# Daniel-Lin-S/decode_tonal_langauge

Hardware: AMD Instinct MI355X
Metric: mel-frames/sec (train step) SynthesisModelCNN, 128ch x 400t batch256 (higher is better)
Workload: dtype f32; 1 GPU; SynthesisModelCNN 128ch x 400t -> 80 mel, 4 tones x 2 syllables, L=5, global batch 256 (strong scaling: 256 windows on rank 0), dropout 0.5, NAdam, 1,376,768,720 params; per_gpu_batch=256, global_batch=256, parallelism=dp1, init=drawn on every rank

## Files before the change

decode_tonal_langauge_amd/_cnnrnn_classifier_train_engine.py:

```python
from __future__ import annotations

from typing import Optional

import torch
import torch.nn as nn

from . import _kernels
from ._classifier_engine import C_A, C_B, C_FIRST, K7, Conv7Trunk, geometry, lstm_pack, lstm_pack_buffers
from ._classifier_train_engine import SUPPORTED, ClassifierTrainEngine, check_common, refuse
from ._conv_stack import ConvStack
from ._launch import r4
from ._lib import EPI_MASK, EPI_STORE, LOAD_DIRECT, LOAD_V, LOAD_Y, check, ptr

def lstm2_input_index(b: int, ch: int, s: int, w: int, B: int, tq: int, W: int, channels: int = C_B):
    f = (ch * tq + s) * W + w
    return (f // (channels * W)) * B + b, f % (channels * W)


def check_supported(model) -> None:
    from .models.deep_classifiers import CNNRNNClassifier
    if not isinstance(model, CNNRNNClassifier):
        refuse(f"model {type(model).__name__}")
    tq = geometry(model.input_channels, model.input_length, model.lstm1.hidden_size)["tq"]
    check_common(model, [m.negative_slope for m in model.modules() if isinstance(m, nn.LeakyReLU)], float(model.conv_block3[5].p),
# ... 162 lines not shown
        rows, nhex, cin, cout = S * Tp, S * Tp // 6, st.cin, st.cout
        f32 = dict(dtype=torch.float32, device=self._dev)
        src, Gs = self.P[st.idx - 1], self.G[st.idx]
        tag = f"conv{st.idx}_wgrad"
        fwd_tag = "conv3a_fwd" if st.idx == 2 else "conv3b_fwd"
        kept = self._v7_of == (self.generation, fwd_tag)
        V0, V1 = (self._hex_view(v, cin, nhex) for v in self.V7)
        ev = self._tick(tag + "_xform")
        if not kept:
            check(self.lib.tl_wino63_xform2(ptr(src), ptr(V0), ptr(V1), rows, Tp, st.tin, cin, src.shape[1], cin, self._stream()),
                  "tl_wino63_xform2")
            self._v7_of = (self.generation, fwd_tag)
        Y = self._hex_view(self.Y7, cout, nhex)
        check(self.lib.tl_wino63_ydz(ptr(Gs), ptr(Y), rows, Tp, st.tout, cout, Gs.shape[1], cout, self._stream()), "tl_wino63_ydz")
        if ev:
            ev[1].record()
        sk = self._splitk((cin // 64) * (cout // 64), (rows + 35) // 36, 4096)
        slab = torch.empty(3, sk, 8 * cin, cout, **f32)
        bias_part = torch.empty(sk, cout, **f32)
        ev = self._tick(tag)
        for s, (V, a_hex) in enumerate(((V0, 0), (V1, 0), (V0, 1))):
            self._tn(fn="tl_conv3_wino63v_tn", A=ptr(V), B=ptr(Y), slab=ptr(slab[s]), Krows=rows, A_rows=V.shape[0],
                     B_rows=Y.shape[0], Mdim=cin, Ndim=cout, lda=cin, ldb=cout, ldc=cout, J=3, Tp=Tp, splitk=sk,
                     slab_stride=8 * cin * cout, loader=LOAD_Y, Tvalid=st.tout, a_hex=a_hex,
                     colsum=ptr(bias_part) if s == 0 else None)
        if ev:
            ev[1].record()
        n = 8 * cin * cout
        ev = self._tick(tag + "_reduce")
        red = torch.empty(8 * cin, cout, **f32) if sk > 1 else None
        g3 = torch.empty(cout, cin, 3, **f32)
        gw7 = gw.view(cout, cin, K7)
        for s in range(3):
            if sk > 1:
                self._permute(slab[s], red, (1, 1, 1, n), (0, 0, 0, 1), nz=sk, zs=n)
            check(self.lib.tl_wino63_wgrad_finalize(ptr(red if sk > 1 else slab[s]), ptr(g3), cout, cin, cout, self._stream()),
                  "tl_wino63_wgrad_finalize")
            nt = min(3, K7 - 3 * s)
            gw7[:, :, 3 * s:3 * s + nt].copy_(g3[:, :, :nt])
        self._permute(bias_part, gb, (1, 1, 1, cout), (0, 0, 0, 1), nz=sk, zs=cout)
        if ev:
            ev[1].record()

    def _dgrad7(self, st, w: torch.Tensor) -> None:
        S, Tp = self.S, self.Tp
        rows, nhex, cin, cout = S * Tp, S * Tp // 6, st.cin, st.cout
        Gs, out = self.G[st.idx], self.G[st.idx - 1]
# ... 95 lines not shown
```

decode_tonal_langauge_amd/_conv_stack.py:

```python
from __future__ import annotations

from typing import List

import torch

from . import _kernels, _lib
from ._launch import LaunchTimers, launch_nt, launch_tn, permute_reduce, r4
from ._lib import (EPI_C1WGRAD, EPI_GY, EPI_LRELU, EPI_MASK, EPI_MASKY, EPI_POOL, EPI_POOLV, LOAD_DIRECT, LOAD_UNPOOL, LOAD_V,
                   LOAD_Y, check, ptr)


class _Stage:

    def __init__(self, idx, cin, cout, k, pool, tin, tp_in):
        self.idx, self.cin, self.cout, self.k, self.pool = idx, cin, cout, k, pool
        self.tin, self.tp_in = tin, tp_in
        self.tc = tin - k + 1
        self.tout = self.tc // 2 if pool else self.tc
        self.tp_out = tp_in // 2 if pool else tp_in


class ConvStack(LaunchTimers):
    F63_CAPABLE = True

# ... 16 lines not shown
        self.tp1 = max(align, (self.tout1 + align - 1) // align * align)
        _kernels.validate()
        self.wino63 = (self.F63_CAPABLE and _kernels.get("wino") == "6"
                       and self._f63_covers(stage_defs, n_timepoints))
        tp1_default = self.tp1
        if self.wino63:
            self.tp1 = (self.tout1 + 11) // 12 * 12
        self.f63_yprod = (self.wino63 and _kernels.get("f63_yprod") != "0" and stage_defs[0][0] % 256 == 0
                          and self.tp1 >= 12)
        self.f63_yprod3 = (self.wino63 and _kernels.get("f63_yprod") != "0" and stage_defs[1][0] % 256 == 0)
        self.stages: List[_Stage] = []
        cin, tin, tp = self.c1, self.tout1, self.tp1
        for i, (cout, k, pool) in enumerate(stage_defs[1:], start=2):
            st = _Stage(i, cin, cout, k, pool, tin, tp)
            if st.tout < 1:
                raise ValueError("n_timepoints too small for the conv stack")
            if self.wino63 and i == 3:
                st.tp_out = tp1_default // 4
            self.stages.append(st)
            cin, tin, tp = cout, st.tout, st.tp_out
        self.gy4 = self._gy_applies()
        st3 = self.stages[1] if len(self.stages) >= 2 else None
        self.f63_seq16 = bool(self.wino63 and self.f63_yprod and self.f63_yprod3 and self.gy4
                              and _kernels.get("f63_yprod") == "1" and -(-st3.tc // 6) <= 16 < st3.tp_in // 6)
        self.lat = tin
        self.tp5 = tp
        self.ld5 = r4(conv_channels)
        mode = _kernels.get("wino")
        self.wino43 = mode != "0"
        self.store_p1 = _kernels.get("store_p1") == "1"
        self.fuse_c1 = True
        self.wino_vout = True
        self.tn_bm = 0
        self._gy_A = None
        self._vhalo = {}
        self._B = None
        self.generation = 0

    def _alloc(self, B: int, dev) -> bool:
        if self._B == B and self._dev == dev:
            return False
        self._B, self._dev = B, dev
        self.S = B * self.C
        self._v_ready = {}
        self._gy_A = None
        self._vhalo = {}
        self._alloc_rows()
# ... 142 lines not shown
        Pout = self.P.get(st.idx) if (st.idx != 2 or self.store_p1) else None
        kw = dict(A=ptr(V), A_rows=V.shape[0], lda=V.shape[2], loader=LOAD_V, Bw=ptr(wp), bias=ptr(bia), out=ptr(Pout),
                  M=S * st.tp_in, N=st.cout, K=st.cin, ldb=st.cin, ldo=Pout.shape[1] if Pout is not None else st.cout, J=3,
                  row_shift=0, Tp=st.tp_in, slope=self.slope, obits=ptr(self.bits[st.idx]), osign=ptr(self.sbits[st.idx]),
                  ld_obits=st.cout // 32, Tvalid=2 * st.tout)
        if st.idx == 2:
            rows_out = S * st.tp_out
            Vn = self._v_hex_buffer(self.V, 2, rows_out, st.cout)
            ntm = -(-(S * st.tp_in) // self._nt63_rows())
            halo = self._halo_buffer(2, ntm, st.cout)
            kw.update(epilogue=EPI_POOLV, vout=ptr(Vn), vhalo=ptr(halo), vout_quads=Vn.shape[0], ld_vout=Vn.shape[2])
            self._nt(tag="conv2_fwd", fn="tl_conv3_wino63v_nt", **kw)
            check(self.lib.tl_wino63_v_fixup(ptr(Vn), ptr(halo), rows_out // 6, ntm, st.tp_out, st.cout, Vn.shape[2],
                                             self._stream()), "tl_wino63_v_fixup")
            self._v_ready[2] = Vn
        else:
            if Pout is None:
                raise RuntimeError("F(6,3) stage 3 writes pooled rows: its output buffer was not allocated")
            kw.update(epilogue=EPI_POOL, out_tp=st.tp_out)
            if self._seq16(st):
                kw.update(M=S * 96, Tp=96, a_hps_extra=st.tp_in // 6 - 16)
            self._nt(tag="conv3_fwd", fn="tl_conv3_wino63v_nt", **kw)

    def _stage_wgrad63(self, st, gw, gb) -> None:
        S = self.S
        f32 = dict(dtype=torch.float32, device=self._dev)
        rows_in = S * st.tp_in
        nd = st.cout
        ldg = nd
        V = self._v_ready[st.idx - 1]
        tiles = (st.cin // 64) * (nd // 64)
        sk = self._splitk(tiles, (rows_in + 35) // 36, 4096)
        slab = torch.empty(sk, 8 * st.cin, ldg, **f32)
        bias_part = torch.empty(sk, nd, **f32)
        if (st.idx == 3 and self.f63_yprod3 and self._y_ready.get(3) != self.generation):
            Gs = self.G[3]
            Y3 = self._v_hex_buffer(self.Yt, 3, rows_in, nd)
            Vd3 = self._vd3_buffer(rows_in, nd)
            ev = self._tick("conv3_yvd")
            check(self.lib.tl_wino63_unpool_yvd(ptr(Gs), ptr(self.bits[3]), ptr(Y3), ptr(Vd3), rows_in, Gs.shape[0], st.tp_in,
                                                st.tp_out, 2 * st.tout, nd, Gs.shape[1], st.cout // 32, nd, self._stream()),
                  "tl_wino63_unpool_yvd")
            if ev:
                ev[1].record()
            self._y_ready[3] = self.generation
            self._vd_ready[3] = self.generation
        if self._y_ready.get(st.idx) == self.generation:
            Y = self.Yt[st.idx]
            self._y_ready[st.idx] = -1
            self._tn(tag=f"conv{st.idx}_wgrad", fn="tl_conv3_wino63v_tn", A=ptr(V), B=ptr(Y), slab=ptr(slab), Krows=rows_in,
                     A_rows=V.shape[0], B_rows=Y.shape[0], Mdim=st.cin, Ndim=nd, lda=V.shape[2], ldb=Y.shape[2], ldc=ldg, J=3,
                     Tp=st.tp_in, splitk=sk, slab_stride=8 * st.cin * ldg, loader=LOAD_Y, Tvalid=2 * st.tout,
                     colsum=ptr(bias_part))
        else:
            Gs = self.G[st.idx]
            Vd = self._v_hex_buffer(self.Vd, st.idx, rows_in, nd)
            self._tn(tag=f"conv{st.idx}_wgrad", fn="tl_conv3_wino63v_tn", A=ptr(V), B=ptr(Gs), slab=ptr(slab), Krows=rows_in,
                     A_rows=V.shape[0], B_rows=Gs.shape[0], Mdim=st.cin, Ndim=nd, lda=V.shape[2], ldb=Gs.shape[1], ldc=ldg, J=3,
                     Tp=st.tp_in, splitk=sk, slab_stride=8 * st.cin * ldg, loader=LOAD_UNPOOL, bbits=ptr(self.bits[st.idx]),
                     ld_bbits=st.cout // 32, Tvalid=2 * st.tout, colsum=ptr(bias_part), vd=ptr(Vd), ld_vd=nd, g_tp=st.tp_out)
            self._vd_ready[st.idx] = self.generation
        self._wino_wgrad_tail(st, slab, bias_part, 8, "tl_wino63_wgrad_finalize", gw, gb)

    def _wino_wgrad_tail(self, st, slab, bias_part, taps, finalize, gw, gb) -> None:
        sk, rows, ldg = slab.shape
        if sk > 1:
            red = torch.empty(rows, ldg, dtype=torch.float32, device=self._dev)
            n = taps * st.cin * ldg
            self._permute(slab, red, (1, 1, 1, n), (0, 0, 0, 1), nz=sk, zs=n)
        else:
            red = slab
        check(getattr(self.lib, finalize)(ptr(red), ptr(gw), st.cout, st.cin, ldg, self._stream()), finalize)
        self._permute(bias_part, gb, (1, 1, 1, st.cout), (0, 0, 0, 1), nz=sk, zs=bias_part.shape[1])

    def _gy_stage(self, st) -> bool:
# ... 435 lines not shown
```

decode_tonal_langauge_amd/_kernels.py:

```python
from __future__ import annotations

import os
from typing import Callable, Dict, Tuple, Union

_Allowed = Union[frozenset, Callable[[str], bool]]


def _int(lo: int, hi: int) -> Callable[[str], bool]:
    def ok(v: str) -> bool:
        try:
            return lo <= int(v) <= hi
        except ValueError:
            return False
    return ok


_B = frozenset({"0", "1"})
KEYS: Dict[str, Tuple[str, _Allowed, str, str]] = {
    "wino": ("TONAL_WINO", frozenset({"6", "4", "0"}), "6",
             "conv2 / conv3: 6 Winograd F(6,3) on pre-transformed operands (F(4,3) V form where the stack does not allow it), "
             "4 the F(4,3) V form, 0 direct MFMA kernels (also the fallback for every shape neither form covers)"),
    "f63_yprod": ("TONAL_F63_YPROD", frozenset({"0", "1", "vd3"}), "1",
                  "F(6,3): the backward operands of stages 2 and 3 (Y2 for both passes of stage 2; Y3) come pre-transformed out of the "
                  "input-gradient epilogue of the stage above; where conv3's valid rows fit 16 hexes of a longer stored sequence, its "
                  "forward and input gradient run on whole-sequence tiles (16 hexes computed), the input gradient on Y3 (vd3: conv3 "
                  "keeps the stored geometry and its input gradient runs on Vd3, which conv4's input gradient writes beside Y3; 0: the "
                  "weight-gradient kernels un-pool and transform the gradient rows themselves and write Vd)"),
    "conv4_dgrad": ("TONAL_CONV4_DGRAD", frozenset({"nt63", "gemm"}), "nt63",
                    "F(6,3): the one-tap stage behind conv3 - nt63: its input gradient on the NT63 kernel, writing Y3 / Vd3 "
                    "(no gradient rows, no tl_wino63_unpool_yvd); gemm: one-tap GEMM + tl_wino63_unpool_yvd"),
    "store_p1": ("TONAL_STORE_P1", _B, "0", "keep the raw pooled rows of stages 1 / 2 beside V, and Vd2 beside Y2 (tests)"),
    "conv7": ("TONAL_CONV7", frozenset({"wino63", "wino63bwd", "direct"}), "wino63",
              "the CNN-RNN classifier's 7-tap convolutions: wino63 three F(6,3) segments forward, direct kernels backward; "
              "wino63bwd the same forward and, in training, both backward passes on F(6,3) as well; direct all direct"),
    "whh_dh": ("TONAL_WHH_DH", _B, "1", "single process: the W_hh NAdam pass also produces the last BPTT product dh_1 = dgates_2 . W_hh "
                                        "(0: a W_hh stream of its own for it)"),
    "whh_stream": ("TONAL_WHH_STREAM", _B, "1", "label LSTM backward: dgates . W_hh as a pure stream of the weight (tl_lstm_gw; 0: the skinny "
                                                "MFMA GEMM with split-K slabs, also the form for more than 8 distinct label rows)"),
    "graph": ("TONAL_GRAPH", _B, "1", "SynthesisLite step replayed as a HIP graph"),
    "lstm_shard": ("TONAL_LSTM_SHARD", _B, "1", "data parallel: label LSTM sharded by gate rows"),
    "hilbert": ("TONAL_HILBERT", frozenset({"auto", "ols", "ols_full", "sym", "taps", "fft"}), "auto",
                "Hilbert bank: force a path (ols band-limited overlap-save, ols_full all 1024 bins per band, sym / taps the "
                "time-domain kernels with / without Hermitian symmetry, fft the DFT-domain form)"),
    "hilbert_f32": ("TONAL_HILBERT_F32", _B, "0", "float32 recordings: fp32 transforms end to end (default: fp64 math)"),
    "butter": ("TONAL_BUTTER", frozenset({"seq", "scan"}), "seq",
               "Butterworth: seq the sequential recurrence (bit-identical to scipy's loop), scan the time-parallel block scan - "
               "zero-phase (up to 9 taps): 2e-8 - 5e-8 from seq, the size of the reference's own rounding, ~20 x faster; "
               "causal=True (up to 8 sections): the first two blocks bit-equal, the rest within a few times scipy's own distance "
               "from long double (1e-16 - 1e-11 by design)"),
# ... 58 lines not shown
```

decode_tonal_langauge_amd/_lib.py:

```python
from __future__ import annotations

import ctypes as C
import os
from typing import Optional

_HERE = os.path.dirname(os.path.abspath(__file__))
LIB_PATH = os.environ.get("TONAL_HIP_LIB", os.path.join(_HERE, "libtonal_hip.so"))

LOAD_DIRECT, LOAD_UNPOOL, LOAD_V = 0, 1, 2
EPI_STORE, EPI_LRELU, EPI_POOL, EPI_MASK, EPI_C1WGRAD, EPI_POOLV, EPI_MASKY, EPI_GY = 0, 1, 2, 3, 4, 5, 6, 7
LOAD_Y = 3


class NtParams(C.Structure):
    _fields_ = [
        ("A", C.c_void_p), ("abits", C.c_void_p), ("Bw", C.c_void_p), ("bias", C.c_void_p), ("aux", C.c_void_p),
        ("out", C.c_void_p), ("obits", C.c_void_p),
        ("M", C.c_int64), ("A_rows", C.c_int64),
        ("N", C.c_int), ("K", C.c_int),
        ("lda", C.c_int), ("ldb", C.c_int), ("ldo", C.c_int), ("ldaux", C.c_int), ("ld_abits", C.c_int),
        ("ld_obits", C.c_int),
        ("J", C.c_int), ("row_shift", C.c_int),
        ("Tp", C.c_int), ("Tvalid", C.c_int), ("Tvalid_in", C.c_int),
        ("slope", C.c_float),
# ... 42 lines not shown
    "tl_wino63_xform2s": (_I, [_P, _P, _P, _L, _I, _I, _I, _I, _I, _I, _P]),
    "tl_conv7_wino63v_dgrad_nt": (_I, [C.POINTER(NtParams), _P]),
    "tl_wino63_unpool_rows6": (_I, [_P, _P, _P, _L, _L, _I, _I, _I, _I, _I, _I, _I, _I, _P]),
    "tl_wino63_weights1": (_I, [_P, _P, _I, _I, _I, _P]),
    "tl_conv1_wino63v_dgrad_nt": (_I, [C.POINTER(NtParams), _P]),
    "tl_comm_unique_id": (_I, [_P]),
    "tl_comm_init": (_I, [C.POINTER(C.c_void_p), _I, _I, _P]),
    "tl_comm_destroy": (_I, [_P]),
    "tl_allreduce": (_I, [_P, _P, _P, _L, _I, _P]),
    "tl_reduce_scatter": (_I, [_P, _P, _P, _L, _P]),
    "tl_all_gather": (_I, [_P, _P, _P, _L, _P]),
    "tl_wino43_wgrad_finalize": (_I, [_P, _P, _I, _I, _I, _P]),
    "tl_wino43_input_transform": (_I, [_P, _P, _L, _I, _I, _I, _I, _P]),
    "tl_conv3_wino43v_nt": (_I, [C.POINTER(NtParams), _P]),
    "tl_wino43_v_fixup": (_I, [_P, _P, _L, _L, _I, _I, _I, _P]),
    "tl_wino43_unpool_transform": (_I, [_P, _P, _P, _L, _L, _I, _I, _I, _I, _I, _I, _P]),
    "tl_conv3_wino43v_tn": (_I, [C.POINTER(TnParams), _P]),
    "tl_wino63_weights": (_I, [_P, _P, _P, _I, _I, _I, _I, _P]),
    "tl_wino63_weights_y": (_I, [_P, _P, _I, _I, _I, _P]),
    "tl_conv3_wino63v_nt": (_I, [C.POINTER(NtParams), _P]),
    "tl_wino63_nt_tile_rows": (_I, []),
    "tl_wino63_v_fixup": (_I, [_P, _P, _L, _L, _I, _I, _I, _P]),
    "tl_conv3_wino63v_tn": (_I, [C.POINTER(TnParams), _P]),
    "tl_wino63_wgrad_finalize": (_I, [_P, _P, _I, _I, _I, _P]),
    "tl_wino63_vd_fixup": (_I, [_P, _P, _L, _L, _I, _I, _I, _P]),
    "tl_wino63_unpool_yvd": (_I, [_P, _P, _P, _P, _L, _L, _I, _I, _I, _I, _I, _I, _I, _P]),
    "tl_conv1_fwd_v6": (_I, [_P, _P, _P, _P, _P, _P, _P, _L, _I, _I, _I, _I, _I, _F, _P]),
    "tl_sizeof_nt_params": (_I, []),
    "tl_sizeof_tn_params": (_I, []),
    "tl_conv1_fwd": (_I, [_P, _P, _P, _P, _P, _P, _L, _I, _I, _I, _I, _I, _F, _P]),
    "tl_conv1_fwd_v": (_I, [_P, _P, _P, _P, _P, _P, _P, _L, _I, _I, _I, _I, _I, _F, _P]),
    "tl_dropout_scale": (_I, [_P, _L, _F, C.c_uint64, _P]),
    "tl_dropout_scale_at": (_I, [_P, _L, _F, C.c_uint64, _L, _P]),
    "tl_conv1_wgrad": (_I, [_P, _P, _P, _P, _I, _L, _I, _I, _I, _I, _I, _P]),
    "tl_permute_reduce": (_I, [_P, _P, C.POINTER(_L), C.POINTER(_L), C.POINTER(_L), _I, _L, _P, _P]),
    "tl_colsum": (_I, [_P, _P, _I, _L, _I, _I, _I, _I, _P]),
    "tl_lstm_cell_fwd": (_I, [_P, _P, _P, _P, _P, _P, _P, _P, _P, _I, _I, _I, _I, _P]),
    "tl_lstm_gw": (_I, [_P, _P, _P, _I, _L, _I, _L, _L, _I, _P]),
    "tl_lstm_infer_seq_fused": (_I, [_P, _L, _P, _P, _P, _P, _I, _I, _I, C.POINTER(C.c_int), _P]),
    "tl_lstm_cell_bwd": (_I, [_P, _P, _P, _P, _P, _P, _P, _P, _P, _I, _I, _I, _P]),
    "tl_lstm_ih_grad": (_I, [_P, _P, _P, _P, _P, _I, _I, _I, _I, _P]),
    "tl_concat_pack": (_I, [_P, _P, _P, _P, _I, _I, _I, _I, _I, _I, _I, _I, _I, _F, C.c_uint64, _L, _P]),
    "tl_concat_unpack_bwd": (_I, [_P, _P, _P, _P, _P, _P, _I, _I, _I, _I, _I, _I, _I, _I, _I, _I, _F, _F,
                                  C.c_uint64, _L, _P]),
    "tl_l1_mcd": (_I, [_P, _P, _P, _P, _I, _I, _I, _I, _F, _P]),
    "tl_nadam": (_I, [_P, _P, _P, _P, _L, _F, _F, _F, _F, _F, _F, _F, _F, _P]),
# ... 131 lines not shown
```

decode_tonal_langauge_amd/csrc/tonal_wino63.hip:

```cpp
#include "tonal_common.h"
#include "tonal_wino43_epi.h"
#include "tonal_wino43v_epi.h"
#include "tonal_wino63_epi.h"
#include "tonal_wino63_kloop.h"
#include <type_traits>

namespace tl {

typedef __attribute__((address_space(3))) void lds_void6_t;
__device__ __forceinline__ void dma16h(__amdgpu_buffer_rsrc_t rs, char* lds_dst, unsigned voff, unsigned soff) {
  __builtin_amdgcn_raw_ptr_buffer_load_lds(rs, (lds_void6_t*)lds_dst, 16, voff, soff, 0, 0);
}

typedef int v6_i32x4 __attribute__((ext_vector_type(4)));
__device__ __forceinline__ v6_i32x4 v6_rsrc_words(const void* base, long long bytes) {
  const unsigned long long a = (unsigned long long)base;
  const long long n = bytes < 0 ? 0 : (bytes < 0x7fffffffLL ? bytes : 0x7fffffffLL);
  return v6_i32x4{(int)(unsigned)a, (int)(unsigned)((a >> 32) & 0xffffu), (int)n, 0x00020000};
}

__device__ __forceinline__ long long v6_at(long long hex, int i, int c, int kc8) {
  return ((((hex >> 1) * kc8 + (c >> 3)) * 8 + i) * 2 + (hex & 1)) * 8 + (c & 7);
}

// ... 1160 lines not shown
  f32x4 d[8];
#pragma unroll
  for (int j = 2; j < 8; ++j) d[j] = *reinterpret_cast<const f32x4*>(v + 16 * j);
  if (t > 0 && (q % hps) != 0) {
    d[0] = *reinterpret_cast<const f32x4*>(halo + ((t - 1) * 2) * (long long)C + c);
    d[1] = *reinterpret_cast<const f32x4*>(halo + ((t - 1) * 2 + 1) * (long long)C + c);
  } else {
    d[0] = d[1] = f32x4{0.f, 0.f, 0.f, 0.f};
  }
  f32x4 o[8];
#pragma unroll
  for (int k = 0; k < 4; ++k) {
    float dd[8], vv[8];
#pragma unroll
    for (int j = 0; j < 8; ++j) dd[j] = d[j][k];
    wino63_bt(dd, vv);
#pragma unroll
    for (int j = 0; j < 8; ++j) o[j][k] = vv[j];
  }
#pragma unroll
  for (int j = 0; j < 8; ++j) *reinterpret_cast<f32x4*>(v + 16 * j) = o[j];
}

__global__ __launch_bounds__(512, 1) void wino63v_tn4y_kernel(const tl_tn_params p, int mtn) {
  constexpr int NA = 4;
  constexpr int QT = 4 * T6_PLANE;
  __shared__ __attribute__((aligned(1024))) float lds[NA * 4 * QT + NA * QT + 256];
  float* As = lds;
  float* Ys = lds + NA * 4 * QT;
  const int tid = threadIdx.x, lane = tid & 63;
  const int wave = __builtin_amdgcn_readfirstlane(tid >> 6);
  const int wm = wave >> 1, wn = wave & 1, lr = lane & 31, lh = lane >> 5;
  const int ntn = p.Ndim / T6_BN;
  const long long tiles = 2LL * mtn * ntn;
  const long long nwg = tiles * p.splitk;
  long long bid = (long long)blockIdx.y * gridDim.x + blockIdx.x;
  {
    const long long q = nwg / 8, r = nwg % 8, x = bid % 8, i = bid / 8;
    bid = (x < r ? x * (q + 1) : r * (q + 1) + (x - r) * q) + i;
  }
  const int z = __builtin_amdgcn_readfirstlane((int)(bid / tiles));
  const int tt = __builtin_amdgcn_readfirstlane((int)(bid % tiles));
  const int mi = __builtin_amdgcn_readfirstlane(tt % (2 * mtn));
  const int th = mi & 1, i0 = 4 * th;
  const int m0 = (mi >> 1) * 256, n0 = __builtin_amdgcn_readfirstlane((tt / (2 * mtn)) * T6_BN);
  const long long hexes_all = p.Krows / 6;
  const long long ksteps_all = (hexes_all + T6_H - 1) / T6_H;
  const long long per = __builtin_amdgcn_readfirstlane((int)((ksteps_all + p.splitk - 1) / p.splitk));
  const long long ks_begin = z * per;
  long long ks_end = ks_begin + per;
  if (ks_end > ksteps_all) ks_end = ksteps_all;
  const int nsteps = ks_end > ks_begin ? (int)(ks_end - ks_begin) : 0;

  f32x16 acc[8];
#pragma unroll
  for (int i = 0; i < 8; ++i)
#pragma unroll
    for (int e = 0; e < 16; ++e) acc[i][e] = 0.f;

  const long long v_h0 = ks_begin * T6_H;
  const int kc8 = p.lda >> 3, kcy = p.ldb >> 3;
  const __amdgpu_buffer_rsrc_t rsV = __builtin_amdgcn_make_buffer_rsrc(
      (void*)(p.A + v_h0 * 8 * (long long)p.lda), 0, clip31((p.A_rows - v_h0) * 8 * (long long)p.lda * 4), 0x00020000);
  const __amdgpu_buffer_rsrc_t rsY = __builtin_amdgcn_make_buffer_rsrc(
      (void*)(p.B + v_h0 * 8 * (long long)p.ldb), 0, clip31((p.B_rows - v_h0) * 8 * (long long)p.ldb * 4), 0x00020000);
  unsigned vvoff[3], vdst[3];
#pragma unroll
  for (int t = 0; t < 3; ++t) {
    const int quarter = (wave * 3 + t) / 6, pc = (wave * 3 + t) % 6;
    const int rho = 4 * pc + (lane >> 4), i = rho / 6, hx = rho % 6;
    const int chunk = (lane & 15) ^ ((hx & 1) << 3);
    vvoff[t] = (unsigned)(v6_at(hx + p.a_hex, i0 + i, m0 + quarter * 64 + chunk * 4, kc8) * 4);
    vdst[t] = (unsigned)((quarter * QT + pc * 256) * 4);
  }
  const bool ypiece = wave < T6_H;
  unsigned yvoff;
  {
    const int rho = 4 * (ypiece ? wave : 0) + (lane >> 4), i = rho / 6, hx = rho % 6;
    const int chunk = (lane & 15) ^ ((hx & 1) << 3);
    yvoff = (unsigned)(v6_at(hx, i0 + i, n0 + chunk * 4, kcy) * 4);
  }
  const unsigned v_step = (unsigned)(T6_H * 8 * p.lda * 4), y_step = (unsigned)(T6_H * 8 * p.ldb * 4);
  auto issue = [&](int step) {
    char* vb = reinterpret_cast<char*>(As) + (step & (NA - 1)) * (4 * QT * 4);
    const unsigned soff = (unsigned)step * v_step;
#pragma unroll
    for (int t = 0; t < 3; ++t) dma16h(rsV, vb + vdst[t], vvoff[t] + soff, 0u);
    char* yb = reinterpret_cast<char*>(Ys) + (ypiece ? ((step & (NA - 1)) * QT + wave * 256) * 4 : NA * QT * 4);
    dma16h(rsY, yb, ypiece ? yvoff + (unsigned)step * y_step : 0xfffffff0u, 0u);
  };
  const int a_off0 = wm * QT + lh * 64 + (lr ^ (lh << 5)), a_off1 = wm * QT + lh * 64 + ((32 + lr) ^ (lh << 5));
  const int b_off = lh * 64 + ((wn * 32 + lr) ^ (lh << 5));
  float fa0[8], fb0[4], fa1[8], fb1[4], fac[8], fbc[4];
  auto load_frag = [&](float (&fa)[8], float (&fb)[4], int buf, int sl) {
    const float* a_s = As + buf * (4 * QT) + sl * 128;
    const float* b_s = Ys + buf * QT + sl * 128 + b_off;
#pragma unroll
    for (int t = 0; t < 4; ++t) {
      fa[t] = a_s[a_off0 + t * T6_PLANE];
      fa[4 + t] = a_s[a_off1 + t * T6_PLANE];
      fb[t] = b_s[t * T6_PLANE];
    }
  };
  auto mfma8 = [&](const float (&fa)[8], const float (&fb)[4]) {
#pragma unroll
    for (int i = 0; i < 8; ++i) acc[i] = __builtin_amdgcn_mfma_f32_32x32x2f32(fa[i], fb[i & 3], acc[i], 0, 0, 0);
  };
#pragma unroll
  for (int i = 0; i < 8; ++i) fac[i] = 0.f;
#pragma unroll
  for (int i = 0; i < 4; ++i) fbc[i] = 0.f;
  const bool summer = p.colsum != nullptr && mi == 0 && wave == 0;
  float bsum = 0.f;
  issue(0);
  issue(1);
  issue(2);
  __builtin_amdgcn_s_waitcnt(0x0078);
  __builtin_amdgcn_s_barrier();
  asm volatile("" ::: "memory");
  for (int s = 0; s < nsteps; ++s) {
    const int buf = s & (NA - 1);
    __builtin_amdgcn_sched_barrier(0);
    issue(s + 3);
    load_frag(fa0, fb0, buf, 0);
    mfma8(fac, fbc);
    load_frag(fa1, fb1, buf, 1);
    mfma8(fa0, fb0);
    load_frag(fac, fbc, buf, 2);
    mfma8(fa1, fb1);
    __builtin_amdgcn_sched_group_barrier(0x100, 6, 0);
#pragma unroll
    for (int t = 0; t < 24; ++t) {
      __builtin_amdgcn_sched_group_barrier(0x008, 1, 0);
      if (t < 4) __builtin_amdgcn_sched_group_barrier(0x010, 1, 0);
      if (t >= 4 && t < 16) __builtin_amdgcn_sched_group_barrier(0x100, 1, 0);
    }
    __builtin_amdgcn_sched_barrier(0);
    if (summer) {
      const float* y1 = Ys + buf * QT + T6_PLANE;
#pragma unroll
      for (int hx = 0; hx < T6_H; ++hx) bsum += y1[hx * 64 + (lane ^ ((hx & 1) << 5))];
    }
    __builtin_amdgcn_s_waitcnt(0x0078);
    __builtin_amdgcn_s_barrier();
    asm volatile("" ::: "memory");
  }
  mfma8(fac, fbc);
  if (summer) p.colsum[(long long)z * p.Ndim + n0 + lane] = bsum;
  float* out = p.slab + (long long)z * p.slab_stride;
  const int col = n0 + wn * 32 + lr;
#pragma unroll
  for (int i = 0; i < 8; ++i)
#pragma unroll
    for (int e = 0; e < 16; ++e) {
      const int m = m0 + wm * 64 + (i >> 2) * 32 + (e & 3) + 8 * (e >> 2) + 4 * lh;
      out[((long long)(i0 + (i & 3)) * p.Mdim + m) * (long long)p.ldc + col] = acc[i][e];
    }
}

__global__ __launch_bounds__(256, 4) void wino63_unpool_yvd_kernel(const float* __restrict__ G, const uint32_t* __restrict__ bits,
                                                                 float* __restrict__ Y, float* __restrict__ Vd, long long nhex,
                                                                 long long g_rows, int hps, int g_tp, int Tvalid, int C, int ldg,
                                                                 int ld_bits, int ldv) {
  const int tpp = C >> 1;
  const long long idx = (long long)blockIdx.x * blockDim.x + threadIdx.x;
// ... 499 lines not shown
  TL_REQUIRE(8LL * p.N * p.ldb * 4 < (1LL << 31), "conv1_wino63v_dgrad_nt: tap set larger than a buffer resource");
  TL_REQUIRE(128LL * 8 * p.lda * 4 + 4LL * p.K < (1LL << 31), "conv1_wino63v_dgrad_nt: tile span too large");
  const long long ntm = (p.M + V6_ROWS - 1) / V6_ROWS;
  const long long nwg = ntm * ((p.N + V6_BN - 1) / V6_BN);
  TL_REQUIRE(nwg < (1LL << 31), "conv1_wino63v_dgrad_nt: grid too large");
  TL_REQUIRE(p.N % 32 == 0 && p.M + V6_ROWS < (1LL << 31), "conv1_wino63v_dgrad_nt: N %% 32 == 0 and M < 2^31 - 768 needed");
  TL_REQUIRE(p.slope >= 0.f && p.slope <= 1.f, "conv1_wino63v_dgrad_nt: LeakyReLU slope must lie in [0, 1]");
  TL_REQUIRE(p.A_rows >= ntm * V6_BH, "conv1_wino63v_dgrad_nt: A must hold whole 128-hex tiles (pad it with zero hexes)");
  TL_REQUIRE(p.a_hps_extra == 0, "conv1_wino63v_dgrad_nt: no compact-M mode (a_hps_extra must be 0)");
  TL_REQUIRE(p.auxbits != nullptr && p.abits != nullptr, "conv1_wino63v_dgrad_nt: needs auxbits (sign) and abits (arg-max) of the stage below");
  TL_REQUIRE(p.out_tp > 0 && p.out_tp <= p.Tp && 2 * p.out_tp >= p.Tvalid_in, "conv1_wino63v_dgrad_nt: out_tp = rows per sequence of the bit arrays (0 < out_tp <= Tp, covering Tvalid_in / 2)");
  TL_REQUIRE(p.ld_abits * 32 >= p.N && p.ld_auxbits * 32 >= p.N && p.Tvalid_in % 2 == 0 && p.Tvalid_in <= 2 * p.Tp, "conv1_wino63v_dgrad_nt: bad abits / auxbits / Tvalid_in");
  TL_REQUIRE(p.vout && p.ld_vout >= p.N && p.ld_vout % 8 == 0 && p.vout_quads >= p.M / 3 && p.vout_quads % 2 == 0,
             "conv1_wino63v_dgrad_nt: needs vout (>= M / 3 hexes, whole pairs, ld_vout %% 8 == 0)");
  TL_REQUIRE((p.vout2 == nullptr) == (p.vhalo == nullptr),
             "conv1_wino63v_dgrad_nt: takes vout2 and vhalo together (Y and Vd) or neither (Y only: the stage below runs its input gradient on Y)");
  TL_REQUIRE(128LL * 8 * p.ld_vout * 4 < (1LL << 31), "conv1_wino63v_dgrad_nt: ld_vout too large");
  const long long ngrid = nwg < 256 ? nwg : 256;
  if (p.vout2 != nullptr) hipLaunchKernelGGL((wino63v_nt_kernel<W_EPI_GY>), dim3((unsigned)ngrid), dim3(512), 0, (hipStream_t)stream, p);
  else hipLaunchKernelGGL((wino63v_nt_kernel<W6_EPI_GY_Y>), dim3((unsigned)ngrid), dim3(512), 0, (hipStream_t)stream, p);
  return check_launch("conv1_wino63v_dgrad_nt");
}

extern "C" int tl_conv3_wino63v_tn(const tl_tn_params* pp, void* stream) {
  using namespace tl;
  TL_REQUIRE(pp != nullptr, "wino63v_tn: null params");
  tl_tn_params p = *pp;
  if (p.splitk < 1) p.splitk = 1;
  if (p.loader == 3) {
    TL_REQUIRE(p.A && p.B && p.slab, "wino63v_tn: null V/Y/slab");
    TL_REQUIRE(p.J == 3 && p.Tp > 0 && p.Tp % 6 == 0 && p.Krows > 0 && p.Krows % p.Tp == 0, "wino63v_tn: loader 3: bad Tp / Krows");
    TL_REQUIRE(p.Krows + 64 < (1LL << 31), "wino63v_tn: more than 2^31 reduction rows");
    TL_REQUIRE(p.Mdim % 256 == 0 && p.Ndim % 64 == 0 && p.lda % 8 == 0 && p.ldb % 8 == 0 && p.lda >= p.Mdim && p.ldb >= p.Ndim &&
               p.ldc >= p.Ndim, "wino63v_tn: loader 3 needs Mdim %% 256, Ndim %% 64, lda / ldb %% 8");
    TL_REQUIRE(p.A_rows % 2 == 0 && p.B_rows % 2 == 0 && p.vd == nullptr, "wino63v_tn: loader 3: whole hex pairs in V and Y, no Vd");
    TL_REQUIRE(p.a_hex == 0 || p.a_hex == 1, "wino63v_tn: loader 3: a_hex must be 0 or 1");
    TL_REQUIRE(p.splitk <= 65535 && (p.splitk == 1 || p.slab_stride >= 8LL * p.Mdim * p.ldc), "wino63v_tn: bad splitk / slab_stride");
    const long long ks = (p.Krows / 6 + T6_H - 1) / T6_H;
    TL_REQUIRE(p.A_rows >= ks * T6_H && p.B_rows >= ks * T6_H, "wino63v_tn: V and Y must hold whole 6-hex K-steps (pad with zero hexes)");
    const long long per3 = (ks + p.splitk - 1) / p.splitk;
    TL_REQUIRE((per3 + 4) * (long long)T6_H * 8 * p.lda * 4 < (1LL << 31) && (per3 + 4) * (long long)T6_H * 8 * p.ldb * 4 < (1LL << 31),
               "wino63v_tn: a reduction split spans more than 2 GB of V or Y: raise splitk");
    const int ntm3 = p.Mdim / 256;
    hipLaunchKernelGGL(wino63v_tn4y_kernel, dim3((unsigned)(2 * ntm3 * (p.Ndim / T6_BN)), (unsigned)p.splitk, 1), dim3(512), 0,
                       (hipStream_t)stream, p, ntm3);
    return check_launch("wino63v_tn (both operands pre-transformed)");
  }
  TL_REQUIRE(p.A && p.B && p.slab && p.bbits, "wino63v_tn: null V/B/bbits/slab");
  TL_REQUIRE(p.a_hex == 0, "wino63v_tn: a_hex needs loader 3 (both operands pre-transformed)");
  TL_REQUIRE(p.J == 3 && p.loader == 1, "wino63v_tn: 3 taps, UNPOOL loader (1) or pre-transformed Y (3)");
  TL_REQUIRE(p.Tp > 0 && p.Tp % 6 == 0 && p.Tvalid % 2 == 0 && p.Tvalid <= p.Tp, "wino63v_tn: Tp %% 6 == 0 and an even Tvalid <= Tp needed");
  TL_REQUIRE(p.Krows > 0 && p.Krows % p.Tp == 0 && p.Mdim > 0 && p.Ndim > 0, "wino63v_tn: bad sizes (Krows must be whole sequences)");
  TL_REQUIRE(p.Krows + 64 < (1LL << 31), "wino63v_tn: more than 2^31 reduction rows");
  TL_REQUIRE(p.Mdim % 128 == 0 && p.Ndim % 64 == 0 && p.lda % 8 == 0 && p.ldb % 4 == 0 && p.A_rows % 2 == 0,
             "wino63v_tn: Mdim %% 128, Ndim %% 64, lda %% 8, ldb %% 4, whole hex pairs in V needed");
  TL_REQUIRE(p.lda >= p.Mdim && p.ldb >= p.Ndim && p.ldc >= p.Ndim, "wino63v_tn: leading dimension too small");
  TL_REQUIRE(p.ld_bbits * 32 >= p.Ndim && p.ld_bbits % 2 == 0, "wino63v_tn: bbits row too short / odd");
  TL_REQUIRE(p.splitk <= 65535, "wino63v_tn: splitk too large");
  TL_REQUIRE(p.splitk == 1 || p.slab_stride >= 8LL * p.Mdim * p.ldc, "wino63v_tn: slab_stride smaller than 8*Mdim*ldc");
  const int g_tp = p.g_tp > 0 ? p.g_tp : p.Tp / 2;
  TL_REQUIRE(2 * g_tp >= p.Tvalid, "wino63v_tn: g_tp must cover the valid pooled rows");
  TL_REQUIRE(p.B_rows >= (p.Krows / p.Tp) * (long long)g_tp && p.B_rows < (1LL << 30), "wino63v_tn: G holds fewer rows than sequences x g_tp");
  const long long ksteps_all = (p.Krows / 6 + T6_H - 1) / T6_H;
  TL_REQUIRE(p.A_rows >= (ksteps_all + 3) * T6_H, "wino63v_tn: V must hold whole 6-hex K-steps and three more (pad it with zero hexes)");
  const long long per = (ksteps_all + p.splitk - 1) / p.splitk;
  TL_REQUIRE((per + 4) * (long long)T6_H * 8 * p.lda * 4 < (1LL << 31), "wino63v_tn: a reduction split spans more than 2 GB of V: raise splitk");
  TL_REQUIRE((per + 6) * 3LL * T6_H * p.ldb * 4 < (1LL << 31), "wino63v_tn: a reduction split spans more than 2 GB of G: raise splitk");
  TL_REQUIRE(p.vd == nullptr || (p.ld_vd >= p.Ndim && p.ld_vd % 8 == 0), "wino63v_tn: ld_vd must cover Ndim (multiple of 8)");
// ... 42 lines not shown
```

include/tonal_hip.h:

```cpp
#ifndef TONAL_HIP_H
#define TONAL_HIP_H
#include <stdint.h>

#ifdef __cplusplus
extern "C" {
#endif

#define TL_OK 0
#define TL_EINVAL (-1)
#define TL_ELAUNCH (-2)
#define TL_ENODEV (-3)

const char* tl_last_error(void);
int tl_version(void);
int tl_device_count(void);

typedef struct {
  const float* A; const uint32_t* abits; const float* Bw; const float* bias; const float* aux;
  float* out; uint32_t* obits;
  int64_t M;
  int64_t A_rows;
  int N, K;
  int lda, ldb, ldo, ldaux, ld_abits, ld_obits;
  int J;
// ... 26 lines not shown
  float* colsum;
  float* vd; int ld_vd;
  int part;
  int bm;
  int g_tp;
  int a_hex;
} tl_tn_params;
int tl_gemm_tn_window(const tl_tn_params* p, void* stream);

int tl_wino43_weights(const float* w, float* fwd, float* dgr, int O, int I, int ld_f, int ld_d, void* stream);
int tl_wino43_wgrad_finalize(const float* red, float* gw, int O, int I, int ld, void* stream);
int tl_wino43_input_transform(const float* P, float* V, int64_t rows, int Tp, int C, int ldp, int ldv, void* stream);
int tl_conv3_wino43v_nt(const tl_nt_params* p, void* stream);
int tl_wino43_v_fixup(float* V, const float* vhalo, int64_t quads, int64_t tiles, int Tq, int C, int ldv, void* stream);
int tl_wino43_unpool_transform(const float* G, const uint32_t* bits, float* V, int64_t conv_rows, int64_t g_rows, int Tp,
                               int Tvalid, int C, int ldg, int ld_bits, int ldv, void* stream);
int tl_conv3_wino43v_tn(const tl_tn_params* p, void* stream);
int tl_wino63_weights(const float* w, float* fwd, float* dgr, int O, int I, int ld_f, int ld_d, void* stream);
int tl_wino63_weights_y(const float* w, float* dgy, int O, int I, int ld_d, void* stream);
int tl_conv3_wino63v_nt(const tl_nt_params* p, void* stream);
int tl_wino63_nt_tile_rows(void);
int tl_wino63_v_fixup(float* V, const float* vhalo, int64_t hexes, int64_t tiles, int Tq, int C, int ldv, void* stream);
int tl_conv3_wino63v_tn(const tl_tn_params* p, void* stream);
int tl_wino63_wgrad_finalize(const float* red, float* gw, int O, int I, int ld, void* stream);
int tl_wino63_vd_fixup(float* Vd, const float* vhalo, int64_t hexes, int64_t tiles, int hexes_per_seq, int C, int ldv, void* stream);
int tl_wino63_unpool_yvd(const float* G, const uint32_t* bits, float* Y, float* Vd, int64_t conv_rows, int64_t g_rows, int Tp,
                         int g_tp, int Tvalid, int C, int ldg, int ld_bits, int ldv, void* stream);
int tl_conv1_fwd_v6(const float* x, const float* w, const float* b, float* P, float* V, uint32_t* bits, uint32_t* sign,
                    int64_t S, int T, int ktaps, int C1, int Tp, int Tout, float slope, void* stream);
int tl_wino63_xform2(const float* P, float* V0, float* V1, int64_t rows, int Tp, int Tvalid, int C, int ldp, int ldv, void* stream);
int tl_wino63_weights7(const float* w, float* fwd, int O, int I, int taps, void* stream);
int tl_conv7_wino63v_nt(const tl_nt_params* p, void* stream);
int tl_wino63_ydz(const float* G, float* Y, int64_t rows, int Tp, int Tvalid, int C, int ldg, int ldv, void* stream);
int tl_wino63_xform2s(const float* P, float* V0, float* V1, int64_t rows, int Tp, int Tvalid, int shift, int C, int ldp, int ldv,
                      void* stream);
int tl_conv7_wino63v_dgrad_nt(const tl_nt_params* p, void* stream);
int tl_wino63_unpool_rows6(const float* G, const uint32_t* bits, float* A, int64_t rows, int64_t g_rows, int Tp, int g_tp, int Tvalid,
                           int C, int ldg, int ld_bits, int lda, int pad, void* stream);
int tl_wino63_weights1(const float* w, float* taps, int O, int I, int ldb, void* stream);
int tl_conv1_wino63v_dgrad_nt(const tl_nt_params* p, void* stream);
int tl_comm_unique_id(void* id128);
int tl_comm_init(void** comm, int rank, int nranks, const void* id128);
int tl_comm_destroy(void* comm);
int tl_allreduce(void* comm, const float* send, float* recv, int64_t count, int op, void* stream);
int tl_reduce_scatter(void* comm, const float* send, float* recv, int64_t recv_count, void* stream);
int tl_all_gather(void* comm, const float* send, float* recv, int64_t send_count, void* stream);
// ... 255 lines not shown
```

Before: 1323 mel-frames/s.

## Skip zero-padded hexes in F(6,3) weight-gradient K loop

Adds a compact-K variant of the pre-transformed Winograd F(6,3) weight-gradient kernel. Its K loop iterates only over the ceil(valid rows/6) hexes per sequence that can hold a nonzero Y, skipping the pad hexes between sequences by adjusting buffer offsets at each K-step. The split-k count is recomputed from the compact step count. The old full-hex behaviour stays available under a new 'allhex' setting, and the conv7 wgrad path passes Tvalid=Tp so it keeps the full loop. In exchange the kernel does more per-step offset arithmetic and must pad V/Y so the last compact step lands in zero hexes.

```diff
diff --git a/decode_tonal_langauge_amd/_cnnrnn_classifier_train_engine.py b/decode_tonal_langauge_amd/_cnnrnn_classifier_train_engine.py
--- a/decode_tonal_langauge_amd/_cnnrnn_classifier_train_engine.py
+++ b/decode_tonal_langauge_amd/_cnnrnn_classifier_train_engine.py
@@ -208,7 +208,7 @@
         for s, (V, a_hex) in enumerate(((V0, 0), (V1, 0), (V0, 1))):
             self._tn(fn="tl_conv3_wino63v_tn", A=ptr(V), B=ptr(Y), slab=ptr(slab[s]), Krows=rows, A_rows=V.shape[0],
                      B_rows=Y.shape[0], Mdim=cin, Ndim=cout, lda=cin, ldb=cout, ldc=cout, J=3, Tp=Tp, splitk=sk,
-                     slab_stride=8 * cin * cout, loader=LOAD_Y, Tvalid=st.tout, a_hex=a_hex,
+                     slab_stride=8 * cin * cout, loader=LOAD_Y, Tvalid=Tp, a_hex=a_hex,
                      colsum=ptr(bias_part) if s == 0 else None)
         if ev:
             ev[1].record()
diff --git a/decode_tonal_langauge_amd/_conv_stack.py b/decode_tonal_langauge_amd/_conv_stack.py
--- a/decode_tonal_langauge_amd/_conv_stack.py
+++ b/decode_tonal_langauge_amd/_conv_stack.py
@@ -62,7 +62,7 @@
         self.gy4 = self._gy_applies()
         st3 = self.stages[1] if len(self.stages) >= 2 else None
         self.f63_seq16 = bool(self.wino63 and self.f63_yprod and self.f63_yprod3 and self.gy4
-                              and _kernels.get("f63_yprod") == "1" and -(-st3.tc // 6) <= 16 < st3.tp_in // 6)
+                              and _kernels.get("f63_yprod") in ("1", "allhex") and -(-st3.tc // 6) <= 16 < st3.tp_in // 6)
         self.lat = tin
         self.tp5 = tp
         self.ld5 = r4(conv_channels)
@@ -251,6 +251,11 @@
                 kw.update(M=S * 96, Tp=96, a_hps_extra=st.tp_in // 6 - 16)
             self._nt(tag="conv3_fwd", fn="tl_conv3_wino63v_nt", **kw)
 
+    @staticmethod
+    def _wgrad63_ksteps(S: int, tp: int, tvalid: int) -> int:
+        hps, hc = tp // 6, -(-tvalid // 6)
+        return -(-S * (hc if 6 <= hc < hps else hps) // 6)
+
     def _stage_wgrad63(self, st, gw, gb) -> None:
         S = self.S
         f32 = dict(dtype=torch.float32, device=self._dev)
@@ -259,7 +264,9 @@
         ldg = nd
         V = self._v_ready[st.idx - 1]
         tiles = (st.cin // 64) * (nd // 64)
-        sk = self._splitk(tiles, (rows_in + 35) // 36, 4096)
+        tvalid = st.tp_in if _kernels.get("f63_yprod") == "allhex" else 2 * st.tout
+        on_y = self._y_ready.get(st.idx) == self.generation or (st.idx == 3 and self.f63_yprod3)
+        sk = self._splitk(tiles, self._wgrad63_ksteps(S, st.tp_in, tvalid if on_y else st.tp_in), 4096)
         slab = torch.empty(sk, 8 * st.cin, ldg, **f32)
         bias_part = torch.empty(sk, nd, **f32)
         if (st.idx == 3 and self.f63_yprod3 and self._y_ready.get(3) != self.generation):
@@ -279,7 +286,7 @@
             self._y_ready[st.idx] = -1
             self._tn(tag=f"conv{st.idx}_wgrad", fn="tl_conv3_wino63v_tn", A=ptr(V), B=ptr(Y), slab=ptr(slab), Krows=rows_in,
                      A_rows=V.shape[0], B_rows=Y.shape[0], Mdim=st.cin, Ndim=nd, lda=V.shape[2], ldb=Y.shape[2], ldc=ldg, J=3,
-                     Tp=st.tp_in, splitk=sk, slab_stride=8 * st.cin * ldg, loader=LOAD_Y, Tvalid=2 * st.tout,
+                     Tp=st.tp_in, splitk=sk, slab_stride=8 * st.cin * ldg, loader=LOAD_Y, Tvalid=tvalid,
                      colsum=ptr(bias_part))
         else:
             Gs = self.G[st.idx]
diff --git a/decode_tonal_langauge_amd/_kernels.py b/decode_tonal_langauge_amd/_kernels.py
--- a/decode_tonal_langauge_amd/_kernels.py
+++ b/decode_tonal_langauge_amd/_kernels.py
@@ -20,11 +20,13 @@
     "wino": ("TONAL_WINO", frozenset({"6", "4", "0"}), "6",
              "conv2 / conv3: 6 Winograd F(6,3) on pre-transformed operands (F(4,3) V form where the stack does not allow it), "
              "4 the F(4,3) V form, 0 direct MFMA kernels (also the fallback for every shape neither form covers)"),
-    "f63_yprod": ("TONAL_F63_YPROD", frozenset({"0", "1", "vd3"}), "1",
+    "f63_yprod": ("TONAL_F63_YPROD", frozenset({"0", "1", "vd3", "allhex"}), "1",
                   "F(6,3): the backward operands of stages 2 and 3 (Y2 for both passes of stage 2; Y3) come pre-transformed out of the "
                   "input-gradient epilogue of the stage above; where conv3's valid rows fit 16 hexes of a longer stored sequence, its "
                   "forward and input gradient run on whole-sequence tiles (16 hexes computed), the input gradient on Y3 (vd3: conv3 "
-                  "keeps the stored geometry and its input gradient runs on Vd3, which conv4's input gradient writes beside Y3; 0: the "
+                  "keeps the stored geometry and its input gradient runs on Vd3, which conv4's input gradient writes beside Y3; "
+                  "allhex: as 1, but the K loops of the two weight gradients run over every stored hex of a sequence instead of the "
+                  "ceil(valid rows / 6) that can hold a nonzero Y - 34 for 33, 17 for 16 at T = 400; 0: the "
                   "weight-gradient kernels un-pool and transform the gradient rows themselves and write Vd)"),
     "conv4_dgrad": ("TONAL_CONV4_DGRAD", frozenset({"nt63", "gemm"}), "nt63",
                     "F(6,3): the one-tap stage behind conv3 - nt63: its input gradient on the NT63 kernel, writing Y3 / Vd3 "
diff --git a/decode_tonal_langauge_amd/_lib.py b/decode_tonal_langauge_amd/_lib.py
--- a/decode_tonal_langauge_amd/_lib.py
+++ b/decode_tonal_langauge_amd/_lib.py
@@ -88,6 +88,7 @@
     "tl_wino63_nt_tile_rows": (_I, []),
     "tl_wino63_v_fixup": (_I, [_P, _P, _L, _L, _I, _I, _I, _P]),
     "tl_conv3_wino63v_tn": (_I, [C.POINTER(TnParams), _P]),
+    "tl_wino63v_tn_compact_hexes": (_I, [C.POINTER(TnParams)]),
     "tl_wino63_wgrad_finalize": (_I, [_P, _P, _I, _I, _I, _P]),
     "tl_wino63_vd_fixup": (_I, [_P, _P, _L, _L, _I, _I, _I, _P]),
     "tl_wino63_unpool_yvd": (_I, [_P, _P, _P, _P, _L, _L, _I, _I, _I, _I, _I, _I, _I, _P]),
diff --git a/decode_tonal_langauge_amd/csrc/tonal_wino63.hip b/decode_tonal_langauge_amd/csrc/tonal_wino63.hip
--- a/decode_tonal_langauge_amd/csrc/tonal_wino63.hip
+++ b/decode_tonal_langauge_amd/csrc/tonal_wino63.hip
@@ -1206,7 +1206,8 @@
   for (int j = 0; j < 8; ++j) *reinterpret_cast<f32x4*>(v + 16 * j) = o[j];
 }
 
-__global__ __launch_bounds__(512, 1) void wino63v_tn4y_kernel(const tl_tn_params p, int mtn) {
+template <bool CK>
+__global__ __launch_bounds__(512, 1) void wino63v_tn4y_kernel(const tl_tn_params p, int mtn, int hc) {
   constexpr int NA = 4;
   constexpr int QT = 4 * T6_PLANE;
   __shared__ __attribute__((aligned(1024))) float lds[NA * 4 * QT + NA * QT + 256];
@@ -1228,7 +1229,7 @@
   const int mi = __builtin_amdgcn_readfirstlane(tt % (2 * mtn));
   const int th = mi & 1, i0 = 4 * th;
   const int m0 = (mi >> 1) * 256, n0 = __builtin_amdgcn_readfirstlane((tt / (2 * mtn)) * T6_BN);
-  const long long hexes_all = p.Krows / 6;
+  const long long hexes_all = CK ? (p.Krows / p.Tp) * hc : p.Krows / 6;
   const long long ksteps_all = (hexes_all + T6_H - 1) / T6_H;
   const long long per = __builtin_amdgcn_readfirstlane((int)((ksteps_all + p.splitk - 1) / p.splitk));
   const long long ks_begin = z * per;
@@ -1242,13 +1243,22 @@
 #pragma unroll
     for (int e = 0; e < 16; ++e) acc[i][e] = 0.f;
 
-  const long long v_h0 = ks_begin * T6_H;
+  long long v_h0 = ks_begin * T6_H;
+  const int ck_gap = CK ? p.Tp / 6 - hc : 0;
+  unsigned ck_h = 0, ck_r = 0;
+  if (CK) {
+    const unsigned g = (unsigned)ks_begin * T6_H, seq0 = g / (unsigned)hc;
+    const long long st0 = (long long)g + (long long)seq0 * ck_gap;
+    ck_h = __builtin_amdgcn_readfirstlane((int)(g - seq0 * (unsigned)hc));
+    ck_r = __builtin_amdgcn_readfirstlane((int)(st0 & 1));
+    v_h0 = st0 - (st0 & 1);
+  }
   const int kc8 = p.lda >> 3, kcy = p.ldb >> 3;
   const __amdgpu_buffer_rsrc_t rsV = __builtin_amdgcn_make_buffer_rsrc(
       (void*)(p.A + v_h0 * 8 * (long long)p.lda), 0, clip31((p.A_rows - v_h0) * 8 * (long long)p.lda * 4), 0x00020000);
   const __amdgpu_buffer_rsrc_t rsY = __builtin_amdgcn_make_buffer_rsrc(
       (void*)(p.B + v_h0 * 8 * (long long)p.ldb), 0, clip31((p.B_rows - v_h0) * 8 * (long long)p.ldb * 4), 0x00020000);
-  unsigned vvoff[3], vdst[3];
+  unsigned vvoff[3], vdst[3], vvodd[3], vhx[3];
 #pragma unroll
   for (int t = 0; t < 3; ++t) {
     const int quarter = (wave * 3 + t) / 6, pc = (wave * 3 + t) % 6;
@@ -1256,22 +1266,69 @@
     const int chunk = (lane & 15) ^ ((hx & 1) << 3);
     vvoff[t] = (unsigned)(v6_at(hx + p.a_hex, i0 + i, m0 + quarter * 64 + chunk * 4, kc8) * 4);
     vdst[t] = (unsigned)((quarter * QT + pc * 256) * 4);
+    if (CK) {
+      vvodd[t] = (unsigned)(v6_at(hx + 1, i0 + i, m0 + quarter * 64 + chunk * 4, kc8) * 4);
+      vhx[t] = (unsigned)hx;
+    }
   }
   const bool ypiece = wave < T6_H;
-  unsigned yvoff;
+  unsigned yvoff, yvodd = 0, yhx = 0;
   {
     const int rho = 4 * (ypiece ? wave : 0) + (lane >> 4), i = rho / 6, hx = rho % 6;
     const int chunk = (lane & 15) ^ ((hx & 1) << 3);
     yvoff = (unsigned)(v6_at(hx, i0 + i, n0 + chunk * 4, kcy) * 4);
+    if (CK) {
+      yvodd = (unsigned)(v6_at(hx + 1, i0 + i, n0 + chunk * 4, kcy) * 4);
+      yhx = (unsigned)hx;
+    }
   }
   const unsigned v_step = (unsigned)(T6_H * 8 * p.lda * 4), y_step = (unsigned)(T6_H * 8 * p.ldb * 4);
+  const unsigned v_pair = (unsigned)(2 * 8 * p.lda * 4), y_pair = (unsigned)(2 * 8 * p.ldb * 4);
+  unsigned vo[3] = {0u, 0u, 0u}, yo = 0u;
+  auto prep = [&]() {
+    if constexpr (CK) {
+      const unsigned pairs = ck_r >> 1;
+      if (ck_h + T6_H > (unsigned)hc) {
+        const unsigned cut = (unsigned)hc - ck_h, ra = ck_r + (unsigned)ck_gap, pairs_a = ra >> 1;
+        const bool odd_b = ck_r & 1, odd_a = ra & 1;
+#pragma unroll
+        for (int t = 0; t < 3; ++t) {
+          const unsigned before = (odd_b ? vvodd[t] : vvoff[t]) + pairs * v_pair;
+          const unsigned after = (odd_a ? vvodd[t] : vvoff[t]) + pairs_a * v_pair;
+          vo[t] = vhx[t] >= cut ? after : before;
+        }
+        const unsigned before = (odd_b ? yvodd : yvoff) + pairs * y_pair, after = (odd_a ? yvodd : yvoff) + pairs_a * y_pair;
+        yo = yhx >= cut ? after : before;
+      } else if (ck_r & 1) {
+#pragma unroll
+        for (int t = 0; t < 3; ++t) vo[t] = vvodd[t] + pairs * v_pair;
+        yo = yvodd + pairs * y_pair;
+      } else {
+#pragma unroll
+        for (int t = 0; t < 3; ++t) vo[t] = vvoff[t] + pairs * v_pair;
+        yo = yvoff + pairs * y_pair;
+      }
+      ck_h += T6_H;
+      ck_r += T6_H;
+      if (ck_h >= (unsigned)hc) {
+        ck_h -= (unsigned)hc;
+        ck_r += (unsigned)ck_gap;
+      }
+    }
+  };
   auto issue = [&](int step) {
     char* vb = reinterpret_cast<char*>(As) + (step & (NA - 1)) * (4 * QT * 4);
-    const unsigned soff = (unsigned)step * v_step;
-#pragma unroll
-    for (int t = 0; t < 3; ++t) dma16h(rsV, vb + vdst[t], vvoff[t] + soff, 0u);
     char* yb = reinterpret_cast<char*>(Ys) + (ypiece ? ((step & (NA - 1)) * QT + wave * 256) * 4 : NA * QT * 4);
-    dma16h(rsY, yb, ypiece ? yvoff + (unsigned)step * y_step : 0xfffffff0u, 0u);
+    if constexpr (CK) {
+#pragma unroll
+      for (int t = 0; t < 3; ++t) dma16h(rsV, vb + vdst[t], vo[t], 0u);
+      dma16h(rsY, yb, ypiece ? yo : 0xfffffff0u, 0u);
+    } else {
+      const unsigned soff = (unsigned)step * v_step;
+#pragma unroll
+      for (int t = 0; t < 3; ++t) dma16h(rsV, vb + vdst[t], vvoff[t] + soff, 0u);
+      dma16h(rsY, yb, ypiece ? yvoff + (unsigned)step * y_step : 0xfffffff0u, 0u);
+    }
   };
   const int a_off0 = wm * QT + lh * 64 + (lr ^ (lh << 5)), a_off1 = wm * QT + lh * 64 + ((32 + lr) ^ (lh << 5));
   const int b_off = lh * 64 + ((wn * 32 + lr) ^ (lh << 5));
@@ -1296,9 +1353,13 @@
   for (int i = 0; i < 4; ++i) fbc[i] = 0.f;
   const bool summer = p.colsum != nullptr && mi == 0 && wave == 0;
   float bsum = 0.f;
+  prep();
   issue(0);
+  prep();
   issue(1);
+  prep();
   issue(2);
+  prep();
   __builtin_amdgcn_s_waitcnt(0x0078);
   __builtin_amdgcn_s_barrier();
   asm volatile("" ::: "memory");
@@ -1325,6 +1386,7 @@
 #pragma unroll
       for (int hx = 0; hx < T6_H; ++hx) bsum += y1[hx * 64 + (lane ^ ((hx & 1) << 5))];
     }
+    prep();
     __builtin_amdgcn_s_waitcnt(0x0078);
     __builtin_amdgcn_s_barrier();
     asm volatile("" ::: "memory");
@@ -1870,6 +1932,13 @@
   return check_launch("conv1_wino63v_dgrad_nt");
 }
 
+static int tn63_compact_hc(const tl_tn_params& p) {
+  if (p.loader != 3 || p.a_hex != 0 || p.Tp <= 0 || p.Tvalid <= 0) return 0;
+  const int hps = p.Tp / 6, hc = (p.Tvalid + 5) / 6;
+  return hc >= 6 && hc < hps ? hc : 0;
+}
+extern "C" int tl_wino63v_tn_compact_hexes(const tl_tn_params* pp) { return pp != nullptr ? tn63_compact_hc(*pp) : 0; }
+
 extern "C" int tl_conv3_wino63v_tn(const tl_tn_params* pp, void* stream) {
   using namespace tl;
   TL_REQUIRE(pp != nullptr, "wino63v_tn: null params");
@@ -1884,14 +1953,29 @@
     TL_REQUIRE(p.A_rows % 2 == 0 && p.B_rows % 2 == 0 && p.vd == nullptr, "wino63v_tn: loader 3: whole hex pairs in V and Y, no Vd");
     TL_REQUIRE(p.a_hex == 0 || p.a_hex == 1, "wino63v_tn: loader 3: a_hex must be 0 or 1");
     TL_REQUIRE(p.splitk <= 65535 && (p.splitk == 1 || p.slab_stride >= 8LL * p.Mdim * p.ldc), "wino63v_tn: bad splitk / slab_stride");
+    const int ntm3 = p.Mdim / 256;
+    const dim3 grid3((unsigned)(2 * ntm3 * (p.Ndim / T6_BN)), (unsigned)p.splitk, 1);
+    if (const int hc = tn63_compact_hc(p)) {
+      const long long gap = p.Tp / 6 - hc;
+      const long long ksc = ((p.Krows / p.Tp) * hc + T6_H - 1) / T6_H;
+      const long long last = ksc * T6_H - 1;
+      TL_REQUIRE(p.A_rows > last + last / hc * gap && p.B_rows > last + last / hc * gap,
+                 "wino63v_tn: compact K: the compact hexes past the last sequence must land in zero pad hexes of V and Y "
+                 "(compact hex g lies at stored hex g + g / hc * (Tp / 6 - hc): pad both to hold the last 6-hex K-step)");
+      const long long per3 = (ksc + p.splitk - 1) / p.splitk;
+      const long long span = (per3 + 4) * T6_H;
+      const long long stored = span + (span / hc + 2) * gap + 1;
+      TL_REQUIRE(stored * 8 * p.lda * 4 < (1LL << 31) && stored * 8 * p.ldb * 4 < (1LL << 31),
+                 "wino63v_tn: a reduction split spans more than 2 GB of V or Y: raise splitk");
+      hipLaunchKernelGGL(wino63v_tn4y_kernel<true>, grid3, dim3(512), 0, (hipStream_t)stream, p, ntm3, hc);
+      return check_launch("wino63v_tn (both operands pre-transformed, compact K)");
+    }
     const long long ks = (p.Krows / 6 + T6_H - 1) / T6_H;
     TL_REQUIRE(p.A_rows >= ks * T6_H && p.B_rows >= ks * T6_H, "wino63v_tn: V and Y must hold whole 6-hex K-steps (pad with zero hexes)");
     const long long per3 = (ks + p.splitk - 1) / p.splitk;
     TL_REQUIRE((per3 + 4) * (long long)T6_H * 8 * p.lda * 4 < (1LL << 31) && (per3 + 4) * (long long)T6_H * 8 * p.ldb * 4 < (1LL << 31),
                "wino63v_tn: a reduction split spans more than 2 GB of V or Y: raise splitk");
-    const int ntm3 = p.Mdim / 256;
-    hipLaunchKernelGGL(wino63v_tn4y_kernel, dim3((unsigned)(2 * ntm3 * (p.Ndim / T6_BN)), (unsigned)p.splitk, 1), dim3(512), 0,
-                       (hipStream_t)stream, p, ntm3);
+    hipLaunchKernelGGL(wino63v_tn4y_kernel<false>, grid3, dim3(512), 0, (hipStream_t)stream, p, ntm3, 0);
     return check_launch("wino63v_tn (both operands pre-transformed)");
   }
   TL_REQUIRE(p.A && p.B && p.slab && p.bbits, "wino63v_tn: null V/B/bbits/slab");
diff --git a/include/tonal_hip.h b/include/tonal_hip.h
--- a/include/tonal_hip.h
+++ b/include/tonal_hip.h
@@ -72,6 +72,7 @@
 int tl_wino63_nt_tile_rows(void);
 int tl_wino63_v_fixup(float* V, const float* vhalo, int64_t hexes, int64_t tiles, int Tq, int C, int ldv, void* stream);
 int tl_conv3_wino63v_tn(const tl_tn_params* p, void* stream);
+int tl_wino63v_tn_compact_hexes(const tl_tn_params* p);
 int tl_wino63_wgrad_finalize(const float* red, float* gw, int O, int I, int ld, void* stream);
 int tl_wino63_vd_fixup(float* Vd, const float* vhalo, int64_t hexes, int64_t tiles, int hexes_per_seq, int C, int ldv, void* stream);
 int tl_wino63_unpool_yvd(const float* G, const uint32_t* bits, float* Y, float* Vd, int64_t conv_rows, int64_t g_rows, int Tp,
```

New measurement: 1330 mel-frames/s (median of 6 runs). No clear change (+0.6%).
